# nyashiki/nshogi-engine

Hardware: NVIDIA B200
Metric: nn_leaf_evals_per_sec_batch256 (higher is better)
Workload: dtype bf16

## Files before the change

### nshogi-engine_b200/csrc/trunk_common.cuh

```cuda
#pragma once
#include <cuda_bf16.h>
#include <cuda_runtime.h>
#include <stdint.h>

#include "cache_device.cuh"
#include "decode_device.cuh"
#include "epilogue.cuh"
#include "nsb_internal.h"
#include "pack_device.cuh"
#include "umma.cuh"

namespace nsb {

constexpr int kThreads = 384;
constexpr int kEpiThreads = 256;
constexpr int kEpiWarps = kEpiThreads / 32;
constexpr uint32_t kEpiBar = 1;

constexpr int kFcPrefetch = 27;

__device__ __forceinline__ uint4 plane_bits(uint4 f) {
    uint32_t s0 = f.x;
    uint32_t s1 = (f.y & 0x7FFFFFFFu) | (f.z << 31);
    uint32_t s2 = (f.z >> 1) & 0x1FFFFu;
    if ((f.z >> 24) & 1u) {
        const uint32_t r0 = __brev(s2), r1 = __brev(s1), r2 = __brev(s0);
        s0 = __funnelshift_r(r0, r1, 15);
        s1 = __funnelshift_r(r1, r2, 15);
        s2 = r2 >> 15;
    }
    const float v = __uint_as_float(f.w);
    const uint32_t hi = (uint32_t)f32_to_bf16_bits(v);
    const float rest = v - __uint_as_float(hi << 16);
    const uint32_t lo = (rest == rest && (hi & 0x7F80u) != 0x7F80u) ? (uint32_t)f32_to_bf16_bits(rest) : 0u;
    return make_uint4(s0, s1, s2, hi | (lo << 16));
}

__device__ __forceinline__ unsigned long long* eval_timeline(const EvalArgs& a) {
#ifdef NSB_DIAG
    return a.timeline;
#else
    (void)a;
    return nullptr;
#endif
}

__device__ __forceinline__ int eval_count(const EvalArgs& a) { return a.count ? __ldg(a.count) : a.n; }
__device__ __forceinline__ int eval_index(const EvalArgs& a, int li, int n_eff) {
    return li < n_eff ? (a.index ? __ldg(a.index + li) : li) : -1;
}

template <int NPOS, int SPITCH, int GUARD, int NT = kEpiThreads>
__device__ __forceinline__ void expand_features(const DeviceNet& net, const EvalArgs& a, int n_eff, int li0, uint4* featS,
                                                uint8_t* stem_buf, int et, unsigned long long* tl,
                                                uint32_t bar = kEpiBar) {
    const int IN = net.in_channels, stem_chunks = 2 * net.stem_steps;
    if (a.positions != nullptr) {
        const int pos = et >> 5, lane = et & 31;
        if (pos < NPOS) {
            uint4* mine = featS + pos * IN;
            const int b = eval_index(a, li0 + pos, n_eff);
            if (b >= 0) {
                pack_position_warp(a.positions + b, lane, mine, [&](int c, uint4 f) { mine[c] = plane_bits(f); });
            } else {
                for (int c = lane; c < IN; c += 32) mine[c] = make_uint4(0, 0, 0, 0);
            }
        }
    } else {
        for (int i = et; i < NPOS * IN; i += NT) {
            const int pos = i / IN, c = i - pos * IN;
            const int b = eval_index(a, li0 + pos, n_eff);
            uint4 f = make_uint4(0, 0, 0, 0);
            if (b >= 0) f = __ldg(reinterpret_cast<const uint4*>(a.features) + (size_t)b * IN + c);
            featS[i] = plane_bits(f);
        }
    }
    if (tl) tl[9] = clock64();
    named_bar_sync(bar, NT);
    if (tl) tl[3] = clock64();
    for (int item = et; item < NPOS * stem_chunks * 9; item += NT) {
        const int pos = item / (stem_chunks * 9);
        const int r2 = item - pos * (stem_chunks * 9);
        const int j = r2 / 9, row = r2 - j * 9;
        const int bit0 = 9 * row, wi = bit0 >> 5, sh = bit0 & 31;
        uint32_t field[8], val[8];
#pragma unroll
        for (int e = 0; e < 8; ++e) {
            const int c = j * 8 + e;
            uint4 f = make_uint4(0, 0, 0, 0);
            const int src = stem_source_channel(c, IN);
            if (src >= 0) f = featS[pos * IN + src];
            const uint32_t lo = wi == 0 ? f.x : (wi == 1 ? f.y : f.z);
            const uint32_t hi = wi == 0 ? f.y : (wi == 1 ? f.z : 0u);
            field[e] = __funnelshift_r(lo, hi, sh);
            val[e] = c < IN ? (f.w & 0xFFFFu) : (f.w >> 16);
        }
        uint8_t* dst = stem_buf + (size_t)((j * SPITCH + GUARD + pos * 100 + row * 10) * 16);
#pragma unroll
        for (int col = 0; col < 9; ++col) {
            uint32_t w[4];
#pragma unroll
            for (int e2 = 0; e2 < 4; ++e2) {
                const uint32_t a0 = val[2 * e2] & (0u - ((field[2 * e2] >> col) & 1u));
                const uint32_t a1 = val[2 * e2 + 1] & (0u - ((field[2 * e2 + 1] >> col) & 1u));
                w[e2] = a0 | (a1 << 16);
            }
            *reinterpret_cast<uint4*>(dst + col * 16) = make_uint4(w[0], w[1], w[2], w[3]);
        }
    }
    if (tl) tl[10] = clock64();
}

template <int COL0>
__device__ __forceinline__ void head_read(uint32_t taddr, float bias, int hp, float* scratch, float* vbuf, int lane) {
#pragma unroll
    for (int j = 0; j < 3; ++j) {
        uint32_t v[32];
        tmem_ld32(taddr + j * 32, v);
        tmem_ld_wait();
        if (lane < 7) {
            float* dst = hp < kPolicyPlanes ? scratch + hp * 81 : vbuf;
            const bool relu = hp == kPolicyPlanes;
#pragma unroll
            for (int i = 0; i < 32; ++i) {
                const int n = COL0 + j * 32 + i;
                if (is_real_slot(n)) {
                    const int pos = n / 100, m = n % 100, t = (m / 10) * 9 + (m % 10);
                    const float x = __uint_as_float(v[i]) + bias;
                    dst[(relu ? pos * 81 : pos * kPolicySize) + t] = relu ? fmaxf(x, 0.f) : x;
                }
            }
        }
    }
}

__device__ __forceinline__ void fc1_prefetch(const DeviceNet& net, int et, float (&wpre)[kFcPrefetch]) {
    const int H = net.hidden;
#pragma unroll
    for (int t = 0; t < kFcPrefetch; ++t) wpre[t] = et < H ? __ldg(net.fc1t + (size_t)t * H + et) : 0.f;
}

template <int NPOS, int NT>
__device__ __forceinline__ void decode_tail(const EvalArgs& a, int n_eff, int li0, float* scratch, const float* wd, int et,
                                            uint32_t bar = kEpiBar) {
    constexpr int NW = NT / 32;
    const int ew = et >> 5, lane = et & 31;
    if (ew < NPOS) {
        const int b = eval_index(a, li0 + ew, n_eff);
        if (b >= 0) {
            const uint32_t mb = __ldg(a.move_off + b), me = __ldg(a.move_off + b + 1);
            const int m = (int)(me - mb);
            const float w = wd[ew * 2 + 0], d = wd[ew * 2 + 1];
            const int rf = a.row_flags ? (int)__ldg(a.row_flags + b) : 0;
            float* row = scratch + ew * kPolicySize;
            float* lout = a.logits_out ? a.logits_out + mb : nullptr;
            bool nan_found;
            if (a.hashes != nullptr) {
                const uint64_t hash = __ldg(a.hashes + b);
                auto store = [&](const float (&v)[kDecodePerLane]) {
                    cache_store_warp_from(a.cache, hash, m, [&](int k) { return v[k]; }, w, d, lane);
                };
                nan_found = a.order_out ? warp_decode_row<true>(row, a.move_idx + mb, m, a.decode_mode, rf, w, d, a.legal_out + mb, lout, lane, row, store)
                                        : warp_decode_row<false>(row, a.move_idx + mb, m, a.decode_mode, rf, w, d, a.legal_out + mb, lout, lane, nullptr, store);
            } else {
                nan_found = a.order_out ? warp_decode_row<true>(row, a.move_idx + mb, m, a.decode_mode, rf, w, d, a.legal_out + mb, lout, lane, row)
                                        : warp_decode_row<false>(row, a.move_idx + mb, m, a.decode_mode, rf, w, d, a.legal_out + mb, lout, lane);
            }
            if (a.nan_flag && lane == 0) a.nan_flag[b] = nan_found ? 1 : 0;
        }
    }
    if (a.order_out != nullptr) {
        named_bar_sync(bar, NT);
        const int pos = ew % NPOS;
        const int b = eval_index(a, li0 + pos, n_eff);
        uint16_t* ostage = reinterpret_cast<uint16_t*>(scratch + pos * kPolicySize + 608);
        if (b >= 0) {
            const uint32_t mb = __ldg(a.move_off + b), me = __ldg(a.move_off + b + 1);
            rank_row_coop(scratch + pos * kPolicySize, (int)(me - mb), ew / NPOS, NW / NPOS, lane, ostage);
        }
        named_bar_sync(bar, NT);
        if (b >= 0) {
            const uint32_t mb = __ldg(a.move_off + b), me = __ldg(a.move_off + b + 1);
            rank_row_copy_out(ostage, (int)(me - mb), ew / NPOS, NW / NPOS, lane, a.order_out + mb);
        }
    }
}

__device__ __forceinline__ int block_steps(const DeviceNet& net, int L, int kc) { return (L == 0 && kc == 1) ? net.stem_steps - 4 : 4; }

template <int NPOS, int NT>
__device__ __forceinline__ void heads_tail_small(const DeviceNet& net, const EvalArgs& a, int n_eff, int li0,
                                                 float* scratch, const float* vbuf, float* red, int et,
                                                 uint32_t bar = kEpiBar) {
    constexpr int NW = NT / 32;
    const int ew = et >> 5, lane = et & 31;
    const int H = net.hidden;
    if (a.policy != nullptr) {
        for (int idx = et; idx < NPOS * kPolicySize; idx += NT) {
            const int pos = idx / kPolicySize, b = eval_index(a, li0 + pos, n_eff);
            if (b >= 0) a.policy[(size_t)b * kPolicySize + (idx - pos * kPolicySize)] = scratch[idx];
        }
    }
    float o[NPOS][2];
#pragma unroll
    for (int pos = 0; pos < NPOS; ++pos) o[pos][0] = o[pos][1] = 0.f;
    for (int h = et; h < H; h += NT) {
        float acc[NPOS];
        const float b1 = __ldg(net.fc1b + h);
#pragma unroll
        for (int pos = 0; pos < NPOS; ++pos) acc[pos] = b1;
#pragma unroll 9
        for (int t = 0; t < 81; ++t) {
            const float w = __ldg(net.fc1t + (size_t)t * H + h);
#pragma unroll
            for (int pos = 0; pos < NPOS; ++pos) acc[pos] += w * vbuf[pos * 81 + t];
        }
        const float w0 = __ldg(net.fc2 + h), w1 = __ldg(net.fc2 + H + h);
#pragma unroll
        for (int pos = 0; pos < NPOS; ++pos) {
            const float hid = fmaxf(acc[pos], 0.f);
            o[pos][0] += w0 * hid;
            o[pos][1] += w1 * hid;
        }
    }
#pragma unroll
    for (int pos = 0; pos < NPOS; ++pos)
#pragma unroll
        for (int k = 0; k < 2; ++k) {
            const float s = warp_sum(o[pos][k]);
            if (lane == 0) red[(ew * NPOS + pos) * 2 + k] = s;
        }
    named_bar_sync(bar, NT);
    if (et < NPOS * 2) {
        const int pos = et >> 1, k = et & 1;
        float s = __ldg(net.fc2b + k);
#pragma unroll
        for (int qq = 0; qq < NW; ++qq) s += red[(qq * NPOS + pos) * 2 + k];
        const float val = 1.0f / (1.0f + expf(-s));
        red[NW * NPOS * 2 + pos * 2 + k] = val;
        const int b = eval_index(a, li0 + pos, n_eff);
        if (b >= 0) (k == 0 ? a.win : a.draw)[b] = val;
    }
    if (a.move_off != nullptr) {
        named_bar_sync(bar, NT);
        decode_tail<NPOS, NT>(a, n_eff, li0, scratch, red + NW * NPOS * 2, et, bar);
    }
    named_bar_sync(bar, NT);
}

template <int NPOS>
__device__ __forceinline__ void heads_tail(const DeviceNet& net, const EvalArgs& a, int n_eff, int li0, float* scratch,
                                           const float* vbuf, float* red, const float (&wpre)[kFcPrefetch], int et,
                                           unsigned long long* tl) {
    const int ew = et >> 5, lane = et & 31;
    const int H = net.hidden;
    if (a.policy != nullptr) {
        for (int idx = et; idx < NPOS * kPolicySize; idx += kEpiThreads) {
            const int pos = idx / kPolicySize, b = eval_index(a, li0 + pos, n_eff);
            if (b >= 0) a.policy[(size_t)b * kPolicySize + (idx - pos * kPolicySize)] = scratch[idx];
        }
    }
    if (tl) tl[5] = clock64();
    {
        float o[NPOS][2];
#pragma unroll
        for (int pos = 0; pos < NPOS; ++pos) o[pos][0] = o[pos][1] = 0.f;
        if (et < H) {
            const int h = et;
            float acc[NPOS];
            const float b1 = __ldg(net.fc1b + h);
            const float w0 = __ldg(net.fc2 + h), w1 = __ldg(net.fc2 + H + h);
#pragma unroll
            for (int pos = 0; pos < NPOS; ++pos) acc[pos] = b1;
#pragma unroll
            for (int t0 = 0; t0 < 81; t0 += kFcPrefetch) {
                float w[kFcPrefetch];
#pragma unroll
                for (int t = 0; t < kFcPrefetch; ++t)
                    w[t] = t0 == 0 ? wpre[t] : __ldg(net.fc1t + (size_t)(t0 + t) * H + h);
#pragma unroll
                for (int t = 0; t < kFcPrefetch; ++t)
#pragma unroll
                    for (int pos = 0; pos < NPOS; ++pos) acc[pos] += w[t] * vbuf[pos * 81 + t0 + t];
            }
#pragma unroll
            for (int pos = 0; pos < NPOS; ++pos) {
                const float hid = fmaxf(acc[pos], 0.f);
                o[pos][0] = w0 * hid;
                o[pos][1] = w1 * hid;
            }
        }
#pragma unroll
        for (int pos = 0; pos < NPOS; ++pos)
#pragma unroll
            for (int k = 0; k < 2; ++k) {
                const float s = warp_sum(o[pos][k]);
                if (lane == 0) red[(ew * NPOS + pos) * 2 + k] = s;
            }
        named_bar_sync(kEpiBar, kEpiThreads);
        if (et < NPOS * 2) {
            const int pos = et >> 1, k = et & 1;
            float s = __ldg(net.fc2b + k);
#pragma unroll
            for (int qq = 0; qq < kEpiWarps; ++qq) s += red[(qq * NPOS + pos) * 2 + k];
            const float val = 1.0f / (1.0f + expf(-s));
            red[kEpiWarps * NPOS * 2 + pos * 2 + k] = val;
            const int b = eval_index(a, li0 + pos, n_eff);
            if (b >= 0) (k == 0 ? a.win : a.draw)[b] = val;
        }
    }
    if (tl) tl[6] = clock64();
    if (a.move_off != nullptr) {
        named_bar_sync(kEpiBar, kEpiThreads);
        decode_tail<NPOS, kEpiThreads>(a, n_eff, li0, scratch, red + kEpiWarps * NPOS * 2, et);
    }
    named_bar_sync(kEpiBar, kEpiThreads);
    if (tl) tl[7] = clock64();
}

}
```

### nshogi-engine_b200/csrc/trunk_quad.cu

```cuda
#include <cuda_bf16.h>
#include <cuda_runtime.h>
#include <stdint.h>

#include "trunk_common.cuh"

namespace nsb {

namespace {

struct QuadGeom {
    static constexpr int C = 128;
    static constexpr int KCH = C / 8;
    static constexpr int NGRP = 2;
    static constexpr int NPOS = 2;
    static constexpr int QPOS = NGRP * NPOS;
    static constexpr int NCOLS = NPOS * 96;
    static constexpr int GUARD = 12;
    static constexpr int SPITCH = (GUARD + NCOLS + 11) | 1;
    static constexpr int BUF_BYTES = ((KCH * SPITCH * 16 + 127) / 128) * 128;
    static constexpr int KC64 = C / 64;
    static constexpr int TMEM_COLS = 512;
    static constexpr int A_COL0 = NGRP * NCOLS;
    static constexpr int A_STAGES = 8;
    static constexpr int A_STAGE_COLS = 16;
    static constexpr int THREADS = 512;
    static constexpr int GRP_THREADS = 128;
    static constexpr int EPI_WARPS = GRP_THREADS / 32;
    static constexpr int MMA_WARP = 12;
    static constexpr int NBARS = 2 * A_STAGES + 2;
    static constexpr int SCRATCH_BYTES = ((NPOS * kPolicySize * 4 + 15) / 16) * 16;
    static constexpr int FEAT_BYTES = NPOS * kMaxInChannels * 16;
    static constexpr int VBUF_BYTES = ((NPOS * 81 * 4 + 15) / 16) * 16;
    static constexpr int RED_BYTES = ((EPI_WARPS * NPOS * 2 * 4 + NPOS * 2 * 4 + 15) / 16) * 16;
    static constexpr int GRP_BYTES = 2 * BUF_BYTES;
    static constexpr int OFF_BUF_A = 0;
    static constexpr int OFF_BUF_B = BUF_BYTES;
    static constexpr int OFF_VBUF = NGRP * GRP_BYTES;
    static constexpr int OFF_RED = OFF_VBUF + NGRP * VBUF_BYTES;
    static constexpr int OFF_BARS = OFF_RED + NGRP * RED_BYTES;
    static constexpr int SMEM_BYTES = OFF_BARS + NBARS * 8 + 16 + 128;
    static_assert(BUF_BYTES == 55040, "each group has the duo kernel's activation layout");
    static_assert(SCRATCH_BYTES <= BUF_BYTES && FEAT_BYTES <= BUF_BYTES, "aliases fit into buffer A");
    static_assert(A_COL0 + A_STAGES * A_STAGE_COLS == TMEM_COLS, "two accumulators + the ring fill tensor memory");
    static_assert(SMEM_BYTES <= 232448, "one CTA per SM");
    static_assert(THREADS == 4 * 128, "setmaxnreg acts on whole warpgroups");
    static_assert(128 * 72 + 2 * 128 * 168 + 128 * 40 <= 65536, "re-balanced registers fit the SM");
};

__global__ void __launch_bounds__(QuadGeom::THREADS, 1) trunk_quad_kernel(const DeviceNet net, const EvalArgs a) {
    using G = QuadGeom;
    constexpr int C = G::C;
    extern __shared__ uint8_t smem_raw[];
    uint8_t* smem = reinterpret_cast<uint8_t*>(((uintptr_t)smem_raw + 127) & ~(uintptr_t)127);
    const uint32_t sbase = smem_u32(smem);
    const uint32_t bars = sbase + G::OFF_BARS;
    auto bar_afull = [&](int s) { return bars + 8u * s; };
    auto bar_aempty = [&](int s) { return bars + 8u * (G::A_STAGES + s); };
    const uint32_t bar_act = bars + 8u * (2 * G::A_STAGES);
    const uint32_t bar_acc = bars + 8u * (2 * G::A_STAGES + 1);
    volatile uint32_t* tmem_holder = reinterpret_cast<volatile uint32_t*>(smem + G::OFF_BARS + 8 * G::NBARS);

    const int warp = threadIdx.x >> 5, lane = threadIdx.x & 31;
    const int n_eff = eval_count(a);
    const int quads = (n_eff + G::QPOS - 1) / G::QPOS;
    const int my_passes =
        (int)blockIdx.x < quads ? (quads - (int)blockIdx.x + (int)gridDim.x - 1) / (int)gridDim.x : 0;
    const int NL = net.num_layers;
    const bool stamp = eval_timeline(a) && blockIdx.x == 0;
    unsigned long long* cta_rec = (eval_timeline(a) && blockIdx.x < 1024) ? eval_timeline(a) + 4 * NL + 16 + 3 * blockIdx.x : nullptr;
    if (cta_rec && threadIdx.x == 0) {
        unsigned smid;
        unsigned long long t;
        asm volatile("mov.u32 %0, %%smid;" : "=r"(smid));
        asm volatile("mov.u64 %0, %%globaltimer;" : "=l"(t));
        cta_rec[0] = smid;
        cta_rec[1] = t;
    }

    for (int i = threadIdx.x; i < G::NGRP * G::GRP_BYTES / 16; i += G::THREADS)
        reinterpret_cast<uint4*>(smem)[i] = make_uint4(0, 0, 0, 0);
    if (threadIdx.x == 0) {
        for (int s = 0; s < G::A_STAGES; ++s) {
            mbar_init(bar_afull(s), 4);
            mbar_init(bar_aempty(s), 1);
        }
        mbar_init(bar_act, G::NGRP * G::EPI_WARPS);
        mbar_init(bar_acc, 1);
        fence_mbar_init();
    }
    fence_proxy_async_smem();
    if (warp == G::MMA_WARP) tmem_alloc(smem_u32(const_cast<uint32_t*>(tmem_holder)), G::TMEM_COLS);
    tc_fence_before();
    __syncthreads();
    tc_fence_after();
    const uint32_t tmem_base = *tmem_holder;

    if (warp < 4) {
        setmaxnreg_dec<72>();
        const int row = threadIdx.x;
        const uint32_t lane_addr = tmem_base + ((uint32_t)(warp * 32) << 16) + G::A_COL0;
        const int steps_per_pass = net.stages_per_pass;
        uint32_t slot = 0, phase = 0;
        auto load_stage = [&](uint4 (&dst)[4], const uint4* s) {
            dst[0] = __ldg(s);
            dst[1] = __ldg(s + 1);
            dst[2] = __ldg(s + 256);
            dst[3] = __ldg(s + 257);
        };
        auto store_stage = [&](const uint4 (&buf)[4]) {
            mbar_wait(bar_aempty(slot), phase ^ 1u);
            tc_fence_after();
            asm volatile(
                "tcgen05.st.sync.aligned.32x32b.x16.b32 [%0], "
                "{%1, %2, %3, %4, %5, %6, %7, %8, %9, %10, %11, %12, %13, %14, %15, %16};"
                ::"r"(lane_addr + slot * G::A_STAGE_COLS), "r"(buf[0].x), "r"(buf[0].y), "r"(buf[0].z), "r"(buf[0].w),
                  "r"(buf[1].x), "r"(buf[1].y), "r"(buf[1].z), "r"(buf[1].w), "r"(buf[2].x), "r"(buf[2].y), "r"(buf[2].z),
                  "r"(buf[2].w), "r"(buf[3].x), "r"(buf[3].y), "r"(buf[3].z), "r"(buf[3].w)
                : "memory");
            tmem_st_wait();
            tc_fence_before();
            __syncwarp();
            if (lane == 0) mbar_arrive(bar_afull(slot));
            if (++slot == G::A_STAGES) { slot = 0; phase ^= 1u; }
        };
        const int stages_per_pass = steps_per_pass / 2;
        for (int p = 0; p < my_passes; ++p) {
            const uint4* src = reinterpret_cast<const uint4*>(net.tiles) + (size_t)row * 2;
            uint4 b0[4], b1[4], b2[4];
            int ld = 0, st = 0;
            if (ld < stages_per_pass) { load_stage(b0, src + (size_t)ld * 512); ++ld; }
            if (ld < stages_per_pass) { load_stage(b1, src + (size_t)ld * 512); ++ld; }
            if (ld < stages_per_pass) { load_stage(b2, src + (size_t)ld * 512); ++ld; }
            for (;;) {
                store_stage(b0); ++st;
                if (ld < stages_per_pass) { load_stage(b0, src + (size_t)ld * 512); ++ld; }
                if (st >= stages_per_pass) break;
                store_stage(b1); ++st;
                if (ld < stages_per_pass) { load_stage(b1, src + (size_t)ld * 512); ++ld; }
                if (st >= stages_per_pass) break;
                store_stage(b2); ++st;
                if (ld < stages_per_pass) { load_stage(b2, src + (size_t)ld * 512); ++ld; }
                if (st >= stages_per_pass) break;
            }
        }
    } else if (warp >= G::MMA_WARP) {
        setmaxnreg_dec<40>();
        if (warp == G::MMA_WARP) {
            constexpr uint32_t idesc = make_idesc_bf16_f32(128, G::NCOLS);
            constexpr uint32_t b_lbo = G::SPITCH * 16;
            uint32_t slot = 0, phase = 0, act_phase = 0;
            for (int p = 0; p < my_passes; ++p) {
                for (int L = 0; L < NL; ++L) {
                    mbar_wait(bar_act, act_phase);
                    act_phase ^= 1u;
                    tc_fence_after();
                    if (stamp && p == 0 && lane == 0) eval_timeline(a)[4 * L + 0] = clock64();
                    const bool head = (L == NL - 1);
                    const uint32_t in_buf = sbase + ((L & 1) ? G::OFF_BUF_A : G::OFF_BUF_B);
                    const int ntaps = head ? 1 : 9;
                    for (int kc = 0; kc < G::KC64; ++kc) {
                        const int halves = block_steps(net, L, kc) / 2;
                        for (int tap = 0; tap < ntaps; ++tap) {
                            const int shift = head ? 0 : (tap / 3 - 1) * 10 + (tap % 3 - 1);
                            const uint32_t b_base = in_buf + (uint32_t)((kc * 8 * G::SPITCH + G::GUARD + shift) * 16);
                            if (halves == 2) {
                                const uint32_t s0 = slot, s1 = (slot + 1) % G::A_STAGES;
                                const uint32_t ph1 = s1 == 0 ? phase ^ 1u : phase;
                                mbar_wait(bar_afull(s0), phase);
                                mbar_wait(bar_afull(s1), ph1);
                                tc_fence_after();
                                if (elect_one()) {
                                    const uint32_t b_lo0 = smem_desc_lo(b_base, b_lbo);
                                    const uint32_t b_lo1 = smem_desc_lo(b_base + G::GRP_BYTES, b_lbo);
#pragma unroll
                                    for (int h = 0; h < 2; ++h) {
                                        const uint32_t a_base = tmem_base + G::A_COL0 + (h ? s1 : s0) * G::A_STAGE_COLS;
#pragma unroll
                                        for (int g = 0; g < G::NGRP; ++g)
#pragma unroll
                                            for (int k2 = 0; k2 < 2; ++k2) {
                                                const int k = 2 * h + k2;
                                                umma_bf16_ts(tmem_base + g * G::NCOLS, a_base + k2 * 8,
                                                             smem_desc_from((g ? b_lo1 : b_lo0) + (uint32_t)(2 * k * G::SPITCH), 128),
                                                             idesc, (uint32_t)((kc | tap | k) != 0));
                                            }
                                        umma_commit(bar_aempty(h ? s1 : s0));
                                    }
                                }
                                __syncwarp();
                                slot = (slot + 2) % G::A_STAGES;
                                if (slot < 2) phase ^= 1u;
                                continue;
                            }
                            for (int h = 0; h < halves; ++h) {
                                mbar_wait(bar_afull(slot), phase);
                                tc_fence_after();
                                if (elect_one()) {
                                    const uint32_t a_base = tmem_base + G::A_COL0 + slot * G::A_STAGE_COLS;
                                    const uint32_t b_lo0 = smem_desc_lo(b_base, b_lbo) + (uint32_t)(4 * h * G::SPITCH);
                                    const uint32_t b_lo1 = smem_desc_lo(b_base + G::GRP_BYTES, b_lbo) + (uint32_t)(4 * h * G::SPITCH);
#pragma unroll
                                    for (int g = 0; g < G::NGRP; ++g)
#pragma unroll
                                        for (int k2 = 0; k2 < 2; ++k2)
                                            umma_bf16_ts(tmem_base + g * G::NCOLS, a_base + k2 * 8,
                                                         smem_desc_from((g ? b_lo1 : b_lo0) + (uint32_t)(2 * k2 * G::SPITCH), 128),
                                                         idesc, (uint32_t)((kc | tap | h | k2) != 0));
                                    umma_commit(bar_aempty(slot));
                                }
                                __syncwarp();
                                if (++slot == G::A_STAGES) { slot = 0; phase ^= 1u; }
                            }
                        }
                    }
                    if (elect_one()) umma_commit(bar_acc);
                    __syncwarp();
                    if (stamp && p == 0 && lane == 0) eval_timeline(a)[4 * L + 1] = clock64();
                }
            }
        }
    } else {
        setmaxnreg_inc<168>();
        const int g = (warp - 4) >> 2;
        const int et = threadIdx.x - 128 - g * G::GRP_THREADS;
        const int q = warp & 3;
        const uint32_t bar = kEpiBar + g;
        uint8_t* gsmem = smem + g * G::GRP_BYTES;
        const uint32_t bufA = sbase + g * G::GRP_BYTES + G::OFF_BUF_A, bufB = sbase + g * G::GRP_BYTES + G::OFF_BUF_B;
        float* scratch = reinterpret_cast<float*>(gsmem + G::OFF_BUF_A);
        uint4* featS = reinterpret_cast<uint4*>(gsmem + G::OFF_BUF_A);
        float* vbuf = reinterpret_cast<float*>(smem + G::OFF_VBUF + g * G::VBUF_BYTES);
        float* red = reinterpret_cast<float*>(smem + G::OFF_RED + g * G::RED_BYTES);
        const uint32_t taddr = tmem_base + ((uint32_t)(q * 32) << 16) + g * G::NCOLS;
        const bool stamper = stamp && g == 0 && et == 0;
        EpilogueMask<3> mask0, mask1;
        mask0.init(0, lane);
        mask1.init(96, lane);
        uint32_t acc_phase = 0;
        for (int p = 0; p < my_passes; ++p) {
            const int b0 = ((int)blockIdx.x + p * (int)gridDim.x) * G::QPOS + g * G::NPOS;

            expand_features<G::NPOS, G::SPITCH, G::GUARD, G::GRP_THREADS>(net, a, n_eff, b0, featS, gsmem + G::OFF_BUF_B, et, nullptr, bar);
            named_bar_sync(bar, G::GRP_THREADS);
            for (int i = et; i < G::FEAT_BYTES / 16; i += G::GRP_THREADS) featS[i] = make_uint4(0, 0, 0, 0);
            fence_proxy_async_smem();
            __syncwarp();
            if (lane == 0) mbar_arrive(bar_act);

            for (int L = 0; L < NL - 1; ++L) {
                float bias[4];
#pragma unroll
                for (int k = 0; k < 4; ++k)
                    bias[k] = __ldg(net.bias + (size_t)L * C + 64 * (k >> 1) + 16 * q + 8 * (k & 1) + (lane >> 2));
                mbar_wait(bar_acc, acc_phase);
                acc_phase ^= 1u;
                tc_fence_after();
                if (stamper && p == 0) eval_timeline(a)[4 * L + 2] = clock64();
                const uint32_t out_buf = ((L & 1) ? bufB : bufA) + G::GUARD * 16;
                const bool residual = (L >= 2) && ((L & 1) == 0);
#pragma unroll
                for (int part = 0; part < 2; ++part)
#pragma unroll
                    for (int lb = 0; lb < 2; ++lb) {
                        if (residual)
                            epilogue_half<3, true, 8>(lb, taddr + 96 * part, out_buf, G::SPITCH * 16, 2 * q, 96 * part, bias,
                                                      part ? mask1 : mask0, lane);
                        else
                            epilogue_half<3, false, 8>(lb, taddr + 96 * part, out_buf, G::SPITCH * 16, 2 * q, 96 * part, bias,
                                                       part ? mask1 : mask0, lane);
                    }
                tc_fence_before();
                fence_proxy_async_smem();
                __syncwarp();
                if (lane == 0) mbar_arrive(bar_act);
                if (stamper && p == 0) eval_timeline(a)[4 * L + 3] = clock64();
            }

            const int hp = 7 * q + lane;
            const float hbias = lane < 7 ? __ldg(net.bias + (size_t)(NL - 1) * C + hp) : 0.f;
            mbar_wait(bar_acc, acc_phase);
            acc_phase ^= 1u;
            tc_fence_after();
            head_read<0>(taddr, hbias, hp, scratch, vbuf, lane);
            head_read<96>(taddr + 96, hbias, hp, scratch, vbuf, lane);
            tc_fence_before();
            named_bar_sync(bar, G::GRP_THREADS);
            heads_tail_small<G::NPOS, G::GRP_THREADS>(net, a, n_eff, b0, scratch, vbuf, red, et, bar);
            if (p + 1 < my_passes) {
                for (int i = et; i < G::SCRATCH_BYTES / 16; i += G::GRP_THREADS)
                    reinterpret_cast<uint4*>(scratch)[i] = make_uint4(0, 0, 0, 0);
                named_bar_sync(bar, G::GRP_THREADS);
            }
        }
    }

    tc_fence_before();
    __syncthreads();
    if (cta_rec && threadIdx.x == 0) {
        unsigned long long t;
        asm volatile("mov.u64 %0, %%globaltimer;" : "=l"(t));
        cta_rec[2] = t;
    }
    if (warp == G::MMA_WARP) {
        __syncwarp();
        tmem_dealloc(tmem_base, G::TMEM_COLS);
    }
}

}

int trunk_quad_prepare() {
    cudaError_t e = cudaFuncSetAttribute(trunk_quad_kernel, cudaFuncAttributeMaxDynamicSharedMemorySize, QuadGeom::SMEM_BYTES);
    int nb = 0;
    if (e == cudaSuccess)
        e = cudaOccupancyMaxActiveBlocksPerMultiprocessor(&nb, trunk_quad_kernel, QuadGeom::THREADS, QuadGeom::SMEM_BYTES);
    if (e != cudaSuccess || nb < 1) {
        set_error("trunk quad: cannot configure the kernel: %s (is this an sm_100a device?)", cudaGetErrorString(e));
        return NSB_ERR_NO_DEVICE;
    }
    return 0;
}

int launch_trunk_quad(const DeviceNet& net, const EvalArgs& a, int num_sms, cudaStream_t s) {
    if (a.n <= 0) return 0;
    const int quads = (a.n + QuadGeom::QPOS - 1) / QuadGeom::QPOS;
    const int grid = quads < num_sms ? quads : num_sms;
    trunk_quad_kernel<<<grid, QuadGeom::THREADS, QuadGeom::SMEM_BYTES, s>>>(net, a);
    return 1;
}

}
```

Baseline: 2.573 million.

## Stage fc1 weights into shared memory and prefetch features before setup

After the trunk's last layer, the loader warps copy the fc1 weight matrix with cp.async into the now-idle activation buffers B of both groups. The value head then reads weights from shared memory, each thread handling two hidden units, with vbuf stored transposed so both positions load as one float2. The epilogue warps also load input features into registers before TMEM allocation and barrier setup, so that global latency overlaps with setup. This adds named barriers between loader and epilogue groups and an extra zeroing pass over buffer B between passes, which brings more synchronisation and more register pressure.

```diff
diff --git a/nshogi-engine_b200/csrc/trunk_common.cuh b/nshogi-engine_b200/csrc/trunk_common.cuh
--- a/nshogi-engine_b200/csrc/trunk_common.cuh
+++ b/nshogi-engine_b200/csrc/trunk_common.cuh
@@ -50,10 +50,29 @@
     return li < n_eff ? (a.index ? __ldg(a.index + li) : li) : -1;
 }
 
-template <int NPOS, int SPITCH, int GUARD, int NT = kEpiThreads>
+template <int NPOS, int NT>
+struct FeatureRegs {
+    static constexpr int N = (NPOS * kMaxInChannels + NT - 1) / NT;
+    uint4 f[N];
+};
+
+template <int NPOS, int NT>
+__device__ __forceinline__ void load_features(const DeviceNet& net, const EvalArgs& a, int n_eff, int li0, int et,
+                                              FeatureRegs<NPOS, NT>& r) {
+    if (a.positions != nullptr) return;
+    const int IN = net.in_channels;
+#pragma unroll
+    for (int k = 0; k < FeatureRegs<NPOS, NT>::N; ++k) {
+        const int i = et + k * NT, pos = i / IN, c = i - pos * IN;
+        const int b = i < NPOS * IN ? eval_index(a, li0 + pos, n_eff) : -1;
+        r.f[k] = b >= 0 ? __ldg(reinterpret_cast<const uint4*>(a.features) + (size_t)b * IN + c) : make_uint4(0, 0, 0, 0);
+    }
+}
+
+template <int NPOS, int SPITCH, int GUARD, int NT = kEpiThreads, bool PRE = false>
 __device__ __forceinline__ void expand_features(const DeviceNet& net, const EvalArgs& a, int n_eff, int li0, uint4* featS,
                                                 uint8_t* stem_buf, int et, unsigned long long* tl,
-                                                uint32_t bar = kEpiBar) {
+                                                uint32_t bar = kEpiBar, const FeatureRegs<NPOS, NT>* pre = nullptr) {
     const int IN = net.in_channels, stem_chunks = 2 * net.stem_steps;
     if (a.positions != nullptr) {
         const int pos = et >> 5, lane = et & 31;
@@ -66,6 +85,10 @@
                 for (int c = lane; c < IN; c += 32) mine[c] = make_uint4(0, 0, 0, 0);
             }
         }
+    } else if constexpr (PRE) {
+#pragma unroll
+        for (int k = 0; k < FeatureRegs<NPOS, NT>::N; ++k)
+            if (et + k * NT < NPOS * IN) featS[et + k * NT] = plane_bits(pre->f[k]);
     } else {
         for (int i = et; i < NPOS * IN; i += NT) {
             const int pos = i / IN, c = i - pos * IN;
@@ -111,7 +134,7 @@
     if (tl) tl[10] = clock64();
 }
 
-template <int COL0>
+template <int COL0, bool VT = false>
 __device__ __forceinline__ void head_read(uint32_t taddr, float bias, int hp, float* scratch, float* vbuf, int lane) {
 #pragma unroll
     for (int j = 0; j < 3; ++j) {
@@ -127,7 +150,10 @@
                 if (is_real_slot(n)) {
                     const int pos = n / 100, m = n % 100, t = (m / 10) * 9 + (m % 10);
                     const float x = __uint_as_float(v[i]) + bias;
-                    dst[(relu ? pos * 81 : pos * kPolicySize) + t] = relu ? fmaxf(x, 0.f) : x;
+                    if constexpr (VT)
+                        dst[relu ? t * 2 + pos : pos * kPolicySize + t] = relu ? fmaxf(x, 0.f) : x;
+                    else
+                        dst[(relu ? pos * 81 : pos * kPolicySize) + t] = relu ? fmaxf(x, 0.f) : x;
                 }
             }
         }
@@ -188,10 +214,18 @@
 
 __device__ __forceinline__ int block_steps(const DeviceNet& net, int L, int kc) { return (L == 0 && kc == 1) ? net.stem_steps - 4 : 4; }
 
-template <int NPOS, int NT>
+__device__ __forceinline__ int fc1_rows_lo(int H) {
+    int r = 13760 / H;
+    if (r >= 81) return 81;
+    while ((r * H) & 3) --r;
+    return r;
+}
+
+template <int NPOS, int NT, bool SMEM_FC1 = false>
 __device__ __forceinline__ void heads_tail_small(const DeviceNet& net, const EvalArgs& a, int n_eff, int li0,
                                                  float* scratch, const float* vbuf, float* red, int et,
-                                                 uint32_t bar = kEpiBar) {
+                                                 uint32_t bar = kEpiBar, const float* fc1s_lo = nullptr,
+                                                 const float* fc1s_hi = nullptr, unsigned long long* tl = nullptr) {
     constexpr int NW = NT / 32;
     const int ew = et >> 5, lane = et & 31;
     const int H = net.hidden;
@@ -201,26 +235,69 @@
             if (b >= 0) a.policy[(size_t)b * kPolicySize + (idx - pos * kPolicySize)] = scratch[idx];
         }
     }
+    if (tl) tl[5] = clock64();
     float o[NPOS][2];
 #pragma unroll
     for (int pos = 0; pos < NPOS; ++pos) o[pos][0] = o[pos][1] = 0.f;
-    for (int h = et; h < H; h += NT) {
-        float acc[NPOS];
-        const float b1 = __ldg(net.fc1b + h);
-#pragma unroll
-        for (int pos = 0; pos < NPOS; ++pos) acc[pos] = b1;
+    if constexpr (SMEM_FC1) {
+        static_assert(NPOS == 2 && kMaxHidden <= 2 * NT, "two positions, at most two hidden units per thread");
+        const float2* v2 = reinterpret_cast<const float2*>(vbuf);
+        const int hA = et, hB = et + NT;
+        if (hA < H) {
+            const bool hasB = hB < H;
+            const int rows_lo = fc1_rows_lo(H);
+            const float b1A = __ldg(net.fc1b + hA), b1B = hasB ? __ldg(net.fc1b + hB) : 0.f;
+            const float w0A = __ldg(net.fc2 + hA), w1A = __ldg(net.fc2 + H + hA);
+            const float w0B = hasB ? __ldg(net.fc2 + hB) : 0.f, w1B = hasB ? __ldg(net.fc2 + H + hB) : 0.f;
+            float a0 = b1A, a1 = b1A, c0 = b1B, c1 = b1B;
 #pragma unroll 9
-        for (int t = 0; t < 81; ++t) {
-            const float w = __ldg(net.fc1t + (size_t)t * H + h);
-#pragma unroll
-            for (int pos = 0; pos < NPOS; ++pos) acc[pos] += w * vbuf[pos * 81 + t];
-        }
-        const float w0 = __ldg(net.fc2 + h), w1 = __ldg(net.fc2 + H + h);
-#pragma unroll
-        for (int pos = 0; pos < NPOS; ++pos) {
-            const float hid = fmaxf(acc[pos], 0.f);
-            o[pos][0] += w0 * hid;
-            o[pos][1] += w1 * hid;
+            for (int t = 0; t < rows_lo; ++t) {
+                const float2 v = v2[t];
+                const float wA = fc1s_lo[t * H + hA], wB = hasB ? fc1s_lo[t * H + hB] : 0.f;
+                a0 += wA * v.x;
+                a1 += wA * v.y;
+                c0 += wB * v.x;
+                c1 += wB * v.y;
+            }
+#pragma unroll 9
+            for (int t = rows_lo; t < 81; ++t) {
+                const float2 v = v2[t];
+                const float wA = fc1s_hi[(t - rows_lo) * H + hA], wB = hasB ? fc1s_hi[(t - rows_lo) * H + hB] : 0.f;
+                a0 += wA * v.x;
+                a1 += wA * v.y;
+                c0 += wB * v.x;
+                c1 += wB * v.y;
+            }
+            o[0][0] += w0A * fmaxf(a0, 0.f);
+            o[0][1] += w1A * fmaxf(a0, 0.f);
+            o[1][0] += w0A * fmaxf(a1, 0.f);
+            o[1][1] += w1A * fmaxf(a1, 0.f);
+            if (hasB) {
+                o[0][0] += w0B * fmaxf(c0, 0.f);
+                o[0][1] += w1B * fmaxf(c0, 0.f);
+                o[1][0] += w0B * fmaxf(c1, 0.f);
+                o[1][1] += w1B * fmaxf(c1, 0.f);
+            }
+        }
+    } else {
+        for (int h = et; h < H; h += NT) {
+            float acc[NPOS];
+            const float b1 = __ldg(net.fc1b + h);
+#pragma unroll
+            for (int pos = 0; pos < NPOS; ++pos) acc[pos] = b1;
+#pragma unroll 9
+            for (int t = 0; t < 81; ++t) {
+                const float w = __ldg(net.fc1t + (size_t)t * H + h);
+#pragma unroll
+                for (int pos = 0; pos < NPOS; ++pos) acc[pos] += w * vbuf[pos * 81 + t];
+            }
+            const float w0 = __ldg(net.fc2 + h), w1 = __ldg(net.fc2 + H + h);
+#pragma unroll
+            for (int pos = 0; pos < NPOS; ++pos) {
+                const float hid = fmaxf(acc[pos], 0.f);
+                o[pos][0] += w0 * hid;
+                o[pos][1] += w1 * hid;
+            }
         }
     }
 #pragma unroll
@@ -241,11 +318,13 @@
         const int b = eval_index(a, li0 + pos, n_eff);
         if (b >= 0) (k == 0 ? a.win : a.draw)[b] = val;
     }
+    if (tl) tl[6] = clock64();
     if (a.move_off != nullptr) {
         named_bar_sync(bar, NT);
         decode_tail<NPOS, NT>(a, n_eff, li0, scratch, red + NW * NPOS * 2, et, bar);
     }
     named_bar_sync(bar, NT);
+    if (tl) tl[7] = clock64();
 }
 
 template <int NPOS>
diff --git a/nshogi-engine_b200/csrc/trunk_quad.cu b/nshogi-engine_b200/csrc/trunk_quad.cu
--- a/nshogi-engine_b200/csrc/trunk_quad.cu
+++ b/nshogi-engine_b200/csrc/trunk_quad.cu
@@ -7,6 +7,17 @@
 namespace nsb {
 
 namespace {
+
+constexpr uint32_t kFc1ReadyBar = 3;
+constexpr uint32_t kFc1DoneBar = 4;
+
+__device__ __forceinline__ void stage_f32(uint32_t dst, const float* src, int n, int tid) {
+    const int n4 = n >> 2;
+    for (int i = tid; i < n4; i += 128)
+        asm volatile("cp.async.cg.shared.global [%0], [%1], 16;" ::"r"(dst + 16u * i), "l"(src + 4 * i) : "memory");
+    for (int i = 4 * n4 + tid; i < n; i += 128)
+        asm volatile("cp.async.ca.shared.global [%0], [%1], 4;" ::"r"(dst + 4u * i), "l"(src + i) : "memory");
+}
 
 struct QuadGeom {
     static constexpr int C = 128;
@@ -39,7 +50,8 @@
     static constexpr int OFF_RED = OFF_VBUF + NGRP * VBUF_BYTES;
     static constexpr int OFF_BARS = OFF_RED + NGRP * RED_BYTES;
     static constexpr int SMEM_BYTES = OFF_BARS + NBARS * 8 + 16 + 128;
-    static_assert(BUF_BYTES == 55040, "each group has the duo kernel's activation layout");
+    static_assert(BUF_BYTES == 55040, "each group has the duo kernel's activation layout (and fc1_rows_lo's split)");
+    static_assert(81 * kMaxHidden * 4 <= NGRP * BUF_BYTES - 3 * kMaxHidden * 4, "fc1t fits into the two buffers B");
     static_assert(SCRATCH_BYTES <= BUF_BYTES && FEAT_BYTES <= BUF_BYTES, "aliases fit into buffer A");
     static_assert(A_COL0 + A_STAGES * A_STAGE_COLS == TMEM_COLS, "two accumulators + the ring fill tensor memory");
     static_assert(SMEM_BYTES <= 232448, "one CTA per SM");
@@ -67,6 +79,7 @@
         (int)blockIdx.x < quads ? (quads - (int)blockIdx.x + (int)gridDim.x - 1) / (int)gridDim.x : 0;
     const int NL = net.num_layers;
     const bool stamp = eval_timeline(a) && blockIdx.x == 0;
+    if (stamp && threadIdx.x == 128) eval_timeline(a)[4 * NL + 0] = clock64();
     unsigned long long* cta_rec = (eval_timeline(a) && blockIdx.x < 1024) ? eval_timeline(a) + 4 * NL + 16 + 3 * blockIdx.x : nullptr;
     if (cta_rec && threadIdx.x == 0) {
         unsigned smid;
@@ -75,6 +88,12 @@
         asm volatile("mov.u64 %0, %%globaltimer;" : "=l"(t));
         cta_rec[0] = smid;
         cta_rec[1] = t;
+    }
+
+    FeatureRegs<G::NPOS, G::GRP_THREADS> feat;
+    if (warp >= 4 && warp < G::MMA_WARP) {
+        const int g = (warp - 4) >> 2;
+        load_features(net, a, n_eff, (int)blockIdx.x * G::QPOS + g * G::NPOS, threadIdx.x - 128 - g * G::GRP_THREADS, feat);
     }
 
     for (int i = threadIdx.x; i < G::NGRP * G::GRP_BYTES / 16; i += G::THREADS)
@@ -94,6 +113,7 @@
     __syncthreads();
     tc_fence_after();
     const uint32_t tmem_base = *tmem_holder;
+    if (stamp && threadIdx.x == 128) eval_timeline(a)[4 * NL + 1] = clock64();
 
     if (warp < 4) {
         setmaxnreg_dec<72>();
@@ -142,6 +162,13 @@
                 if (ld < stages_per_pass) { load_stage(b2, src + (size_t)ld * 512); ++ld; }
                 if (st >= stages_per_pass) break;
             }
+            mbar_wait(bar_acc, (uint32_t)((p * NL + NL - 2) & 1));
+            tc_fence_after();
+            const int H = net.hidden, rows_lo = fc1_rows_lo(H);
+            stage_f32(sbase + G::OFF_BUF_B, net.fc1t, rows_lo * H, row);
+            stage_f32(sbase + G::GRP_BYTES + G::OFF_BUF_B, net.fc1t + (size_t)rows_lo * H, (81 - rows_lo) * H, row);
+            asm volatile("cp.async.wait_all;" ::: "memory");
+            named_bar_arrive(kFc1ReadyBar, 128 + G::NGRP * G::GRP_THREADS);
         }
     } else if (warp >= G::MMA_WARP) {
         setmaxnreg_dec<40>();
@@ -233,19 +260,27 @@
         float* red = reinterpret_cast<float*>(smem + G::OFF_RED + g * G::RED_BYTES);
         const uint32_t taddr = tmem_base + ((uint32_t)(q * 32) << 16) + g * G::NCOLS;
         const bool stamper = stamp && g == 0 && et == 0;
+        const float* fc1s_lo = reinterpret_cast<const float*>(smem + G::OFF_BUF_B);
+        const float* fc1s_hi = reinterpret_cast<const float*>(smem + G::GRP_BYTES + G::OFF_BUF_B);
+        if (stamper) eval_timeline(a)[4 * NL + 11] = clock64();
         EpilogueMask<3> mask0, mask1;
         mask0.init(0, lane);
         mask1.init(96, lane);
         uint32_t acc_phase = 0;
         for (int p = 0; p < my_passes; ++p) {
             const int b0 = ((int)blockIdx.x + p * (int)gridDim.x) * G::QPOS + g * G::NPOS;
-
-            expand_features<G::NPOS, G::SPITCH, G::GUARD, G::GRP_THREADS>(net, a, n_eff, b0, featS, gsmem + G::OFF_BUF_B, et, nullptr, bar);
+            unsigned long long* tl = (stamper && p == 0) ? eval_timeline(a) + 4 * NL : nullptr;
+            if (tl) tl[8] = clock64();
+
+            if (p > 0) load_features(net, a, n_eff, b0, et, feat);
+            expand_features<G::NPOS, G::SPITCH, G::GUARD, G::GRP_THREADS, true>(net, a, n_eff, b0, featS, gsmem + G::OFF_BUF_B,
+                                                                                  et, tl, bar, &feat);
             named_bar_sync(bar, G::GRP_THREADS);
             for (int i = et; i < G::FEAT_BYTES / 16; i += G::GRP_THREADS) featS[i] = make_uint4(0, 0, 0, 0);
             fence_proxy_async_smem();
             __syncwarp();
             if (lane == 0) mbar_arrive(bar_act);
+            if (tl) tl[2] = clock64();
 
             for (int L = 0; L < NL - 1; ++L) {
                 float bias[4];
@@ -281,14 +316,21 @@
             mbar_wait(bar_acc, acc_phase);
             acc_phase ^= 1u;
             tc_fence_after();
-            head_read<0>(taddr, hbias, hp, scratch, vbuf, lane);
-            head_read<96>(taddr + 96, hbias, hp, scratch, vbuf, lane);
+            head_read<0, true>(taddr, hbias, hp, scratch, vbuf, lane);
+            head_read<96, true>(taddr + 96, hbias, hp, scratch, vbuf, lane);
             tc_fence_before();
             named_bar_sync(bar, G::GRP_THREADS);
-            heads_tail_small<G::NPOS, G::GRP_THREADS>(net, a, n_eff, b0, scratch, vbuf, red, et, bar);
+            if (tl) tl[4] = clock64();
+            named_bar_sync(kFc1ReadyBar, 128 + G::NGRP * G::GRP_THREADS);
+            heads_tail_small<G::NPOS, G::GRP_THREADS, true>(net, a, n_eff, b0, scratch, vbuf, red, et, bar, fc1s_lo, fc1s_hi, tl);
             if (p + 1 < my_passes) {
+                named_bar_sync(kFc1DoneBar, G::NGRP * G::GRP_THREADS);
+                const int H = net.hidden, rows_lo = fc1_rows_lo(H);
+                const int fc1_vecs = ((g ? 81 - rows_lo : rows_lo) * H + 3) / 4;
                 for (int i = et; i < G::SCRATCH_BYTES / 16; i += G::GRP_THREADS)
                     reinterpret_cast<uint4*>(scratch)[i] = make_uint4(0, 0, 0, 0);
+                for (int i = et; i < fc1_vecs; i += G::GRP_THREADS)
+                    reinterpret_cast<uint4*>(gsmem + G::OFF_BUF_B)[i] = make_uint4(0, 0, 0, 0);
                 named_bar_sync(bar, G::GRP_THREADS);
             }
         }
```

Result: faster. 2.619 million (median of 6 runs) (+1.8%).
